# XiYe20/NPVP

Hardware: AMD Instinct MI355X
Metric: predictor train frames/sec (higher is better)
Workload: dtype f32 (two-term fp16 split of amax-scaled operands, 3 MFMAs per product, fp32 accumulate: fp32-grade; small GEMMs: three-term bf16 split)

## Files before the change

include/npvp_hip.h:

```cpp
#ifndef NPVP_HIP_H
#define NPVP_HIP_H
#include <stddef.h>
#ifdef __cplusplus
extern "C" {
#endif

typedef struct ihipStream_t* npvp_stream_t;

int npvp_version(void);
const char* npvp_last_error(void);
long long npvp_launch_count(void);
void* npvp_stream_create_low_priority(int* least, int* greatest);
int npvp_stream_destroy(void* stream);
void* npvp_event_create(void);
int npvp_event_record(void* event, void* stream);
float npvp_event_elapsed_ms(void* event0, void* event1);
int npvp_event_destroy(void* event);

long long npvp_graph_node_counts(void* graph, long long* counts, long long* memset_bytes, int max_memsets);

long long npvp_gemm_workspace_bytes(int M, int N, int K);
int npvp_gemm_kernel_id(int a_kc, int b_kc, int M, int N, int K, int precision, int has_planes);
int npvp_gemm_route(int a_kc, int b_kc, int M, int N, int K, int precision, int has_planes, int plain_epilogue, int* out4);
int npvp_gemm_f32(int a_kc, int b_kc, int M, int N, int K, const float* A, long long lda, const float* B, long long ldb,
// ... 67 lines not shown
int npvp_layernorm_bwd_reduce_job(const void* workspace, float* dw, float* db, long long rows, int C, int accumulate, void* job);
int npvp_frameln_act_bwd_reduce_job(const void* workspace, float* dw, float* db, int frames, int per_frame, int accumulate, void* job);
int npvp_mlpdw_mid_bwd_reduce_job(const void* workspace, float* gw, float* gb, int frames, int Ch, void* job);
int npvp_sum_rows_multi(const void* jobs, int n, npvp_stream_t stream);

int npvp_layernorm_nchw_fwd(const float* x, const float* w, const float* b, float* out_nchw, float* mean, float* rstd, int frames,
                            int P, int C, float eps, int relu, npvp_stream_t stream);

int npvp_frame_stats(const float* x, const float* add, float* mean, float* rstd, int frames, int T, int per_frame,
                     float eps, npvp_stream_t stream);
int npvp_posfuse_fwd(const float* x, const float* add, const float* beta, const float* gamma, float* y, float* mean,
                     float* rstd, int N, int T, int per_frame, float eps, float* y_amax, npvp_stream_t stream);
int npvp_ln_posfuse_fwd(const float* x, const float* lw, const float* lb, float ln_eps, float* y1, float* ln_mean, float* ln_rstd,
                        const float* add, const float* beta, const float* gamma, float* fused, float* pf_mean, float* pf_rstd,
                        int N, int T, int P, int C, float pf_eps, float* y1_amax, float* fused_amax, npvp_stream_t stream);
int npvp_posfuse_bwd_fused(int N, int T, int per_frame);
int npvp_posfuse_bwd(const float* dy, const float* x, const float* add, const float* gamma, const float* mean,
                     const float* rstd, float* du, float* dyxh, float* dbeta, float* dgamma, int N, int T, int per_frame,
                     int accumulate, void* workspace, long long ws_bytes , npvp_stream_t stream);

int npvp_posfuse_instance_fwd(const float* x, const float* add, const float* beta, const float* gamma, float* y, float* mean,
                              float* rstd, int N, int T, int P, int C, float eps, float* y_amax, npvp_stream_t stream);
int npvp_posfuse_instance_bwd(const float* dy, const float* x, const float* add, const float* gamma, const float* mean,
                              const float* rstd, float* du, float* dyxh, int N, int T, int P, int C, npvp_stream_t stream);

int npvp_frameln_act_fwd(const float* h, const float* mean, const float* rstd, const float* w, const float* b,
                         const float* res, float* out, int frames, int per_frame, float drop_p, unsigned int salt,
                         float dp_p, unsigned int dp_salt, int frames_per_sample, const unsigned long long* seed,
                         float* out_amax, npvp_stream_t stream);
long long npvp_frameln_act_bwd_workspace_bytes(int frames, int per_frame);
// ... 56 lines not shown
int npvp_im2col3x3(const float* in, float* out, int frames, int H, int W, int C, int col2im, npvp_stream_t stream);
long long npvp_dwconv3x3_wgrad_workspace_bytes(int frames, int Ch);
int npvp_dwconv3x3_wgrad(const float* a, const float* dout, float* dwt_db, int frames, int H, int W, int Ch,
                         void* workspace, long long ws_bytes, npvp_stream_t stream);

int npvp_attn_fwd(const float* q, long long ld_q, const float* k, long long ld_k, const float* v, long long ld_v, float* o,
                  long long ld_o, int mode, int dim0, int P, int W, int ws, int Tq, int Tk, int heads, int head_dim,
                  int mask_mode, float drop_p, const unsigned long long* seed, unsigned int salt, float* o_amax,
                  npvp_stream_t stream);
int npvp_attn_bwd(const float* q, long long ld_q, const float* k, long long ld_k, const float* v, long long ld_v,
                  const float* go, long long ld_o, float* dq, long long ld_dq, float* dk, long long ld_dk, float* dv,
                  long long ld_dv, int mode, int dim0, int P, int W, int ws, int Tq, int Tk, int heads, int head_dim,
                  int mask_mode, float drop_p, const unsigned long long* seed, unsigned int salt, float* dq_amax,
                  float* dk_amax , float* dv_amax,
                  npvp_stream_t stream);
int npvp_attn_long_fwd(const float* q, long long ld_q, const float* k, long long ld_k, const float* v, long long ld_v, float* o,
                       long long ld_o, int mode, int dim0, int P, int W, int ws, int Tq, int Tk, int heads, int head_dim,
                       int mask_mode, float drop_p, const unsigned long long* seed, unsigned int salt, float* o_amax,
                       npvp_stream_t stream);
long long npvp_attn_long_bwd_workspace_bytes(int mode, int dim0, int P, int W, int ws, int Tq, int Tk, int heads);
int npvp_attn_long_bwd(const float* q, long long ld_q, const float* k, long long ld_k, const float* v, long long ld_v,
                       const float* go, long long ld_o, float* dq, long long ld_dq, float* dk, long long ld_dk, float* dv,
                       long long ld_dv, int mode, int dim0, int P, int W, int ws, int Tq, int Tk, int heads, int head_dim,
                       int mask_mode, float drop_p, const unsigned long long* seed, unsigned int salt, float* dq_amax,
                       float* dk_amax , float* dv_amax, void* workspace, long long ws_bytes,
                       npvp_stream_t stream);

int npvp_reparam_samples(const float* mu, const float* logvar, float* z, float* eps_out, long long numel, int S,
                         long long sample_base, const unsigned long long* seed, unsigned int salt, npvp_stream_t stream);
int npvp_attn_samples_fwd(const float* q, long long ld_q, const float* k, long long ld_k, const float* v, long long ld_v, float* o,
// ... 155 lines not shown
```

npvp_amd/csrc/attn.hip:

```cpp
#include <cstdio>

#include "common.h"

namespace npvp {

constexpr int HD = 64;
constexpr int LDT = 68;

struct AttnParams {
  const float* q; const float* k; const float* v; const float* go;
  float* o;
  float* dq; float* dk; float* dv;
  long long ld_q, ld_k, ld_v, ld_o;
  long long ld_dq, ld_dk, ld_dv;
  int mode, heads, L, S;
  int P, W, ws, nww, nwin;
  int Tq, Tk;
  int mask_mode;
  float scale;
  unsigned int drop_thresh; float drop_inv_keep; unsigned int salt;
  const unsigned long long* seed;
  long long total;
  float* o_amax; float* dq_amax; float* dk_amax; float* dv_amax;
};

struct AttnRows { int mode, a, b, P, W, ws; float inv_ws; };
__device__ __forceinline__ AttnRows attn_rows(const AttnParams& p, unsigned int g) {
  AttnRows r;
  r.mode = p.mode; r.P = p.P; r.W = p.W; r.ws = p.ws; r.b = 0; r.inv_ws = 0.f;
  if (p.mode == 0) {
    const unsigned int f = g / (unsigned int)p.nwin, win = g - f * (unsigned int)p.nwin;
    const unsigned int qh = win / (unsigned int)p.nww, qw = win - qh * (unsigned int)p.nww;
    r.a = (int)(f * (unsigned int)p.P + qh * (unsigned int)(p.ws * p.W) + qw * (unsigned int)p.ws);
    r.inv_ws = 1.f / (float)p.ws;
  } else {
    const unsigned int n = g / (unsigned int)p.P;
    r.a = (int)n; r.b = (int)(g - n * (unsigned int)p.P);
  }
// ... 13 lines not shown
}
__device__ __forceinline__ float attn_keep(const AttnParams& p, unsigned long long seed, unsigned long long wid, int L, int S, int q, int j) {
  return drop_scale(seed, p.salt, (wid * L + q) * S + j, p.drop_thresh, p.drop_inv_keep);
}
struct AttnWave { int head; AttnRows g; int L, S, Tq, Tk; unsigned long long seed; };
__device__ __forceinline__ AttnWave attn_wave(const AttnParams& p, unsigned int wid) {
  AttnWave aw;
  aw.head = (int)(wid % (unsigned int)p.heads);
  aw.g = attn_rows(p, wid / (unsigned int)p.heads);
  aw.L = p.L; aw.S = p.S;
  aw.Tq = p.mode == 1 ? p.Tq : 0; aw.Tk = p.mode == 1 ? p.Tk : 0;
  aw.seed = (p.seed && p.drop_thresh) ? *p.seed : 0ull;
  return aw;
}

typedef float f32x4_t __attribute__((ext_vector_type(4)));
#define NPVP_MFMA16(A, B, C) __builtin_amdgcn_mfma_f32_16x16x4f32((A), (B), (C), 0, 0, 0)

struct AttnTileR { float v[16]; };
struct AttnTileG { float4 v[4]; };

__device__ __forceinline__ void attn_load_r(AttnTileR& t, const float* src, long long ld, const AttnParams& p, const AttnRows& g,
                                            int nrows, int Tn, int head, int n, int c, int blk) {
  const int r = min(16 * blk + n, nrows - 1);
  const float* q = src + attn_row(g, r, Tn) * ld + head * HD + 16 * c;
#pragma unroll
  for (int s4 = 0; s4 < 4; ++s4) {
    const float4 x = ld4(q + 4 * s4);
    t.v[4 * s4 + 0] = x.x; t.v[4 * s4 + 1] = x.y; t.v[4 * s4 + 2] = x.z; t.v[4 * s4 + 3] = x.w;
  }
// ... 18 lines not shown
    }
  }
}
__device__ __forceinline__ float blk_of(const float4& x, int b) { return b == 0 ? x.x : b == 1 ? x.y : b == 2 ? x.z : x.w; }

__device__ __forceinline__ void attn_mm_rows(f32x4_t (&acc)[4], const float (&a)[4], const AttnTileG& gt) {
#pragma unroll
  for (int b = 0; b < 4; ++b) {
#pragma unroll
    for (int i = 0; i < 4; ++i) acc[b] = NPVP_MFMA16(a[i], blk_of(gt.v[i], b), acc[b]);
  }
}
__device__ __forceinline__ void attn_zero(f32x4_t (&acc)[4]) {
#pragma unroll
  for (int b = 0; b < 4; ++b) acc[b] = f32x4_t{0.f, 0.f, 0.f, 0.f};
}
__device__ __forceinline__ f32x4_t attn_mm_d(const AttnTileR& a, const AttnTileR& b) {
  f32x4_t acc = {0.f, 0.f, 0.f, 0.f};
#pragma unroll
  for (int s = 0; s < 16; ++s) acc = NPVP_MFMA16(a.v[s], b.v[s], acc);
  return acc;
}
__device__ __forceinline__ float quad_max(float v) { v = fmaxf(v, __shfl_xor(v, 16, 64)); return fmaxf(v, __shfl_xor(v, 32, 64)); }
__device__ __forceinline__ float quad_sum(float v) { v += __shfl_xor(v, 16, 64); return v + __shfl_xor(v, 32, 64); }

template <int NK, bool MASK, bool BWD, class KT>
__device__ __forceinline__ void attn_row_block(float (&sc)[NK][4], float (*dp)[4], float& mx, float& inv, KT&& ktile, const AttnTileR& qr,
                                               const AttnTileR* vr, const AttnTileR* gr, float scale, int mask_mode, int L, int S, int q, int c) {
  mx = -INFINITY;
#pragma unroll
// ... 73 lines not shown
    for (int i = 0; i < 4; ++i) {
      sc[kb][i] *= inv;
      if constexpr (STAGED) pm[kb][i] = sc[kb][i] * m[kb][i];
      dp[kb][i] = STAGED ? mul_rounded(dp[kb][i], m[kb][i]) : dp[kb][i] * m[kb][i];
      rs += dp[kb][i] * sc[kb][i];
    }
  return quad_sum(rs);
}

template <int NQ, int NK>
__global__ __launch_bounds__(256) void attn_fwd_mfma_kernel(AttnParams p) {
  const int lane = threadIdx.x & 63, n = lane & 15, c = lane >> 4;
  const long long wid = (long long)blockIdx.x * 4 + (threadIdx.x >> 6);
  if (wid >= p.total) return;
  const AttnWave aw = attn_wave(p, (unsigned int)wid);
  AttnTileR kr[NK];
  AttnTileG vg[NK];
  float am_o = 0.f;
  const unsigned int pk_o = amax_peek_wave(p.o_amax);
#pragma unroll
  for (int kb = 0; kb < NK; ++kb) {
    attn_load_r(kr[kb], p.k, p.ld_k, p, aw.g, aw.S, aw.Tk, aw.head, n, c, kb);
    attn_load_g(vg[kb], p.v, p.ld_v, p, aw.g, aw.S, aw.Tk, aw.head, n, c, kb);
  }
#pragma unroll
  for (int qb = 0; qb < NQ; ++qb) attn_fwd_qblock<NK, false>(p, aw, aw.g, wid, kr, vg, qb, n, c, am_o);
  amax_slot_commit(p.o_amax, am_o, pk_o);
}

template <int NQ, int NK>
// ... 18 lines not shown
  for (int s = (int)ck * chunk; s < s_end; ++s) {
    gq.a = s * nclip + aw.g.a;
#pragma unroll
    for (int qb = 0; qb < NQ; ++qb) attn_fwd_qblock<NK, true>(p, aw, gq, 0ull, kr, vg, qb, n, c, am_o);
  }
  amax_slot_commit(p.o_amax, am_o, pk_o);
}

template <int NQ, int NK>
__global__ __launch_bounds__(256) void attn_bwd_mfma_kernel(AttnParams p) {
  const int lane = threadIdx.x & 63, n = lane & 15, c = lane >> 4;
  const long long wid = (long long)blockIdx.x * 4 + (threadIdx.x >> 6);
  if (wid >= p.total) return;
  const AttnWave aw = attn_wave(p, (unsigned int)wid);
  const AttnRows& g = aw.g; const int head = aw.head, L = aw.L, S = aw.S, Tq = aw.Tq, Tk = aw.Tk;
  AttnTileR kr[NK], vr[NK];
#pragma unroll
  for (int kb = 0; kb < NK; ++kb) {
    attn_load_r(kr[kb], p.k, p.ld_k, p, g, S, Tk, head, n, c, kb);
    attn_load_r(vr[kb], p.v, p.ld_v, p, g, S, Tk, head, n, c, kb);
  }
  float mxs[NQ], invs[NQ], rss[NQ], am_q = 0.f, am_k = 0.f, am_v = 0.f;
  const unsigned int pk_q = amax_peek_wave(p.dq_amax), pk_k = amax_peek_wave(p.dk_amax), pk_v = amax_peek_wave(p.dv_amax);
  AttnTileR qr, gr;
#pragma unroll
  for (int qb = 0; qb < NQ; ++qb) {
    attn_load_r(qr, p.q, p.ld_q, p, g, L, Tq, head, n, c, qb);
    attn_load_r(gr, p.go, p.ld_o, p, g, L, Tq, head, n, c, qb);
    AttnTileG kg[NK];
#pragma unroll
// ... 575 lines not shown
                         long long ld_v, float* o, long long ld_o, float* o_amax) {
  if (ld_q % 4 || ld_k % 4 || ld_v % 4 || ld_o % 4) return attn_fail(who, "row strides must be multiples of 4");
  p.q = q; p.k = k; p.v = v; p.o = o; p.ld_q = ld_q; p.ld_k = ld_k; p.ld_v = ld_v; p.ld_o = ld_o; p.o_amax = o_amax;
  return NPVP_OK;
}
static int attn_bind_bwd(AttnParams& p, const char* who, const float* q, long long ld_q, const float* k, long long ld_k, const float* v,
                         long long ld_v, const float* go, long long ld_o, float* dq, long long ld_dq, float* dk, long long ld_dk, float* dv,
                         long long ld_dv, float* dq_amax, float* dk_amax, float* dv_amax) {
  if (ld_q % 4 || ld_k % 4 || ld_v % 4 || ld_o % 4 || ld_dq % 4 || ld_dk % 4 || ld_dv % 4) return attn_fail(who, "row strides must be multiples of 4");
  p.q = q; p.k = k; p.v = v; p.go = go; p.dq = dq; p.dk = dk; p.dv = dv;
  p.ld_q = ld_q; p.ld_k = ld_k; p.ld_v = ld_v; p.ld_o = ld_o; p.ld_dq = ld_dq; p.ld_dk = ld_dk; p.ld_dv = ld_dv;
  p.dq_amax = dq_amax; p.dk_amax = dk_amax; p.dv_amax = dv_amax;
  return NPVP_OK;
}

}

using namespace npvp;

extern "C" int npvp_attn_fwd(const float* q, long long ld_q, const float* k, long long ld_k, const float* v, long long ld_v,
                             float* o, long long ld_o, int mode, int dim0, int P, int W, int ws, int Tq, int Tk, int heads,
                             int head_dim, int mask_mode, float drop_p, const unsigned long long* seed, unsigned int salt,
                             float* o_amax, hipStream_t stream) {
  AttnParams p = {};
  if (const int rc = attn_setup(p, "attn", mode, heads, head_dim, dim0, P, W, ws, Tq, Tk, mask_mode, drop_p, seed, salt)) return rc;
  NPVP_CHECK_ARG(dim0 > 0, "attn: empty batch");
  if (const int rc = attn_bind_fwd(p, "attn", q, ld_q, k, ld_k, v, ld_v, o, ld_o, o_amax)) return rc;
  const dim3 mg((unsigned)((p.total + 3) / 4)), mb(256);
  const int nq = (p.L + 15) / 16, nk = (p.S + 15) / 16;
  if (nq > 2 || nk > 2) {
    const size_t lds = (size_t)2 * p.S * HD * sizeof(float);
    if (lds > 64 * 1024 && hipFuncSetAttribute((const void*)attn_fwd_generic_kernel, hipFuncAttributeMaxDynamicSharedMemorySize, (int)lds) != hipSuccess)
      return attn_fail("attn", "could not reserve LDS for the generic kernel", NPVP_ERR_LAUNCH);
    NPVP_LAUNCH(attn_fwd_generic_kernel, dim3((unsigned)p.total), dim3(GEN_THREADS), lds, stream, p);
    NPVP_CHECK_LAUNCH();
    return NPVP_OK;
  }
  if (nq == 1 && nk == 1) NPVP_LAUNCH((attn_fwd_mfma_kernel<1, 1>), mg, mb, 0, stream, p);
  else if (nq == 1) NPVP_LAUNCH((attn_fwd_mfma_kernel<1, 2>), mg, mb, 0, stream, p);
  else if (nk == 1) NPVP_LAUNCH((attn_fwd_mfma_kernel<2, 1>), mg, mb, 0, stream, p);
  else NPVP_LAUNCH((attn_fwd_mfma_kernel<2, 2>), mg, mb, 0, stream, p);
// ... 27 lines not shown
  const dim3 mg((unsigned)((p.total + 3) / 4)), mb(256);
  const int nq = (Tq + 15) / 16, nk = (Tk + 15) / 16, ck = (int)chunk;
  if (nq == 1 && nk == 1) NPVP_LAUNCH((attn_samples_fwd_mfma_kernel<1, 1>), mg, mb, 0, stream, p, S, N, ck);
  else if (nq == 1) NPVP_LAUNCH((attn_samples_fwd_mfma_kernel<1, 2>), mg, mb, 0, stream, p, S, N, ck);
  else if (nk == 1) NPVP_LAUNCH((attn_samples_fwd_mfma_kernel<2, 1>), mg, mb, 0, stream, p, S, N, ck);
  else NPVP_LAUNCH((attn_samples_fwd_mfma_kernel<2, 2>), mg, mb, 0, stream, p, S, N, ck);
  NPVP_CHECK_LAUNCH();
  return NPVP_OK;
}

extern "C" int npvp_attn_bwd(const float* q, long long ld_q, const float* k, long long ld_k, const float* v, long long ld_v,
                             const float* go, long long ld_o, float* dq, long long ld_dq, float* dk, long long ld_dk,
                             float* dv, long long ld_dv, int mode, int dim0, int P, int W, int ws, int Tq, int Tk,
                             int heads, int head_dim, int mask_mode, float drop_p, const unsigned long long* seed,
                             unsigned int salt, float* dq_amax, float* dk_amax, float* dv_amax, hipStream_t stream) {
  AttnParams p = {};
  if (const int rc = attn_setup(p, "attn", mode, heads, head_dim, dim0, P, W, ws, Tq, Tk, mask_mode, drop_p, seed, salt)) return rc;
  NPVP_CHECK_ARG(dim0 > 0, "attn_bwd: empty batch");
  if (const int rc = attn_bind_bwd(p, "attn_bwd", q, ld_q, k, ld_k, v, ld_v, go, ld_o, dq, ld_dq, dk, ld_dk, dv, ld_dv, dq_amax, dk_amax, dv_amax))
    return rc;
  const size_t staged1_lds = (size_t)(2 * p.L + p.S) * LDT * sizeof(float) + 2 * 16 * LDX * sizeof(float);
  const dim3 mg((unsigned)((p.total + 3) / 4)), mb(256);
  const int nq = (p.L + 15) / 16, nk = (p.S + 15) / 16;
  if (nq > 2 || nk > 2) {
    const size_t lds = ((size_t)2 * (p.L + p.S) * HD + 3 * (size_t)p.L) * sizeof(float);
    if (lds > 64 * 1024 && hipFuncSetAttribute((const void*)attn_bwd_generic_kernel, hipFuncAttributeMaxDynamicSharedMemorySize, (int)lds) != hipSuccess)
      return attn_fail("attn_bwd", "could not reserve LDS for the generic kernel", NPVP_ERR_LAUNCH);
    NPVP_LAUNCH(attn_bwd_generic_kernel, dim3((unsigned)p.total), dim3(GEN_THREADS), lds, stream, p);
    NPVP_CHECK_LAUNCH();
    return NPVP_OK;
  }
  if (nq == 1 && nk == 1) NPVP_LAUNCH((attn_bwd_mfma_kernel<1, 1>), mg, mb, 0, stream, p);
  else if (nq == 1) NPVP_LAUNCH((attn_bwd_mfma_kernel<1, 2>), mg, mb, 0, stream, p);
// ... 61 lines not shown
```

npvp_amd/csrc/norm.hip:

```cpp
#include "partials.h"
#include <cstring>
#include <cstdlib>

namespace npvp {

template <int NV>
__global__ __launch_bounds__(256) void ln_fwd_kernel(const float* __restrict__ x, const float* __restrict__ w,
                                                     const float* __restrict__ b, float* __restrict__ y,
                                                     float* __restrict__ mean, float* __restrict__ rstd, long long rows,
                                                     float eps, int relu, float* __restrict__ amax) {
  constexpr int C = NV * 256;
  __shared__ float ared[4];
  const unsigned int peek = amax_peek_block(amax);
  const int lane = threadIdx.x & 63;
  float4 ww[NV], bb[NV];
#pragma unroll
  for (int i = 0; i < NV; ++i) { ww[i] = ld4(w + (i * 64 + lane) * 4); bb[i] = ld4(b + (i * 64 + lane) * 4); }
  float am = 0.f;
  for (long long row = (long long)blockIdx.x * 4 + (threadIdx.x >> 6); row < rows; row += (long long)gridDim.x * 4) {
    float4 v[NV];
    float s = 0.f;
#pragma unroll
    for (int i = 0; i < NV; ++i) {
      v[i] = ld4(x + row * C + (i * 64 + lane) * 4);
// ... 279 lines not shown
    if (gt) { const float4 g = ld4(gt + e); o.x *= 1.f + g.x; o.y *= 1.f + g.y; o.z *= 1.f + g.z; o.w *= 1.f + g.w; }
    const float4 b = ld4(bt + e);
    o.x += b.x; o.y += b.y; o.z += b.z; o.w += b.w;
    st4(yf + e, o);
    am = amax4(am, o);
  }
  amax_slot_commit_block(amax, am, ared, peek);
}

__global__ __launch_bounds__(1024) void ln_posfuse_fwd_frame_kernel(const float* __restrict__ x, const float* __restrict__ lw,
                                                                    const float* __restrict__ lb, float ln_eps, float* __restrict__ y1,
                                                                    float* __restrict__ ln_mean, float* __restrict__ ln_rstd,
                                                                    const float* __restrict__ add, const float* __restrict__ beta,
                                                                    const float* __restrict__ gamma, float* __restrict__ fused,
                                                                    float* __restrict__ pf_mean, float* __restrict__ pf_rstd, int T,
                                                                    float pf_eps, float* __restrict__ amax1, float* __restrict__ amax2) {
  constexpr int C = 512, P = 64, PF = P * C;
  __shared__ float red[16];
  __shared__ float ared1[16];
  __shared__ float ared2[16];
  const unsigned int peek1 = amax_peek_block(amax1), peek2 = amax_peek_block(amax2);
  const int f = blockIdx.x, n = f / T, t = f - n * T;
  const int lane = threadIdx.x & 63, wave = threadIdx.x >> 6;
  float4 ww[2], bb[2];
#pragma unroll
  for (int i = 0; i < 2; ++i) { ww[i] = ld4(lw + (i * 64 + lane) * 4); bb[i] = ld4(lb + (i * 64 + lane) * 4); }
  float4 v[4][2];
  float am1 = 0.f, su = 0.f;
#pragma unroll
  for (int r = 0; r < 4; ++r) {
    const int row = wave * 4 + r;
    const long long base = (long long)f * PF + (long long)row * C;
    float s = 0.f;
#pragma unroll
    for (int i = 0; i < 2; ++i) { v[r][i] = ld4(x + base + (i * 64 + lane) * 4); s += (v[r][i].x + v[r][i].y) + (v[r][i].z + v[r][i].w); }
    const float mu = wave_sum(s) * (1.f / C);
    float q = 0.f;
#pragma unroll
// ... 573 lines not shown
    return NPVP_OK;
  }
  NPVP_LAUNCH(frame_stats_kernel, dim3(frames), dim3(512), 0, stream, x, add, mean, rstd, T, per_frame, eps);
  NPVP_CHECK_LAUNCH();
  const long long total4 = (long long)frames * per_frame / 4;
  NPVP_LAUNCH(posfuse_apply_kernel, dim3(ew_blocks(total4, 256)), dim3(256), 0, stream, x, add, beta, gamma,
                     (const float*)mean, (const float*)rstd, y, T, per_frame, total4, amax);
  NPVP_CHECK_LAUNCH();
  return NPVP_OK;
}

extern "C" int npvp_ln_posfuse_fwd(const float* x, const float* lw, const float* lb, float ln_eps, float* y1, float* ln_mean,
                                   float* ln_rstd, const float* add, const float* beta, const float* gamma, float* fused,
                                   float* pf_mean, float* pf_rstd, int N, int T, int P, int C, float pf_eps, float* y1_amax,
                                   float* fused_amax, hipStream_t stream) {
  NPVP_CHECK_ARG(N > 0 && T > 0 && P == 64 && C == 512, "ln_posfuse_fwd: frames of 64 token rows x 512 channels only");
  NPVP_CHECK_ARG(x && lw && lb && y1 && ln_mean && ln_rstd && beta && fused && pf_mean && pf_rstd, "ln_posfuse_fwd: null argument");
  NPVP_LAUNCH(ln_posfuse_fwd_frame_kernel, dim3(N * T), dim3(1024), 0, stream, x, lw, lb, ln_eps, y1, ln_mean, ln_rstd, add,
                     beta, gamma, fused, pf_mean, pf_rstd, T, pf_eps, y1_amax, fused_amax);
  NPVP_CHECK_LAUNCH();
  return NPVP_OK;
}

extern "C" int npvp_posfuse_bwd_fused(int N, int T, int per_frame) {
  if (per_frame % 1024 != 0) return 0;
  const long long blocks = (long long)T * (per_frame / 1024);
  return (blocks >= 128 || N <= 16) ? 1 : 0;
}

extern "C" int npvp_posfuse_bwd(const float* dy, const float* x, const float* add, const float* gamma, const float* mean,
                                const float* rstd, float* du, float* dyxh, float* dbeta, float* dgamma, int N, int T,
                                int per_frame, int accumulate, void* workspace, long long ws_bytes, hipStream_t stream) {
  const int frames = N * T;
  NPVP_CHECK_ARG(N > 0 && T > 0 && per_frame % 4 == 0, "posfuse_bwd: bad shape");
// ... 170 lines not shown
```

npvp_amd/ops.py:

```python
import contextlib
import functools
import os
from collections import namedtuple

import torch

from ._lib import lib, check
from . import sched as _S
from .sched import (_p, _ptr, _stream, _ws, AmaxSlot, GemmProbe, HbmProbe, ProbeEvent, AuxStream, StepContext, current, use, scoped,
                    remember, rng, GradSink, WgradStream, WgradChain, ReduceQueue, RangeGuard)


def amax_of(t, slot=None):
    if slot is not None:
        return slot
    for cand in (t, t._base):
        tag = getattr(cand, "_npvp_amax", None) if cand is not None else None
        if tag is not None and tag[1] == cand._version:
            return tag[0]
    s = AmaxSlot.new(t.device)
    t2 = t if t.dim() == 2 else t.reshape(-1, t.shape[-1])
    if t2.stride(1) != 1:
        t2 = t2.contiguous()
    check(lib().npvp_amax(_ptr(t2), t2.shape[0], t2.shape[1], t2.stride(0), _ptr(s), _stream()), "npvp_amax")
# ... 1067 lines not shown
    return (cfg.ws * cfg.ws, cfg.ws * cfg.ws) if cfg.mode == 0 else (cfg.Tq, cfg.Tk)


def _attn_groups(cfg):
    return cfg.dim0 * (cfg.P // (cfg.ws * cfg.ws)) if cfg.mode == 0 else cfg.dim0 * cfg.P


def _attn_long(cfg):
    return max(_attn_len(cfg)) >= ATTN_LONG_MIN


def _attn_fwd_entry(cfg):
    return (lib().npvp_attn_long_fwd, "npvp_attn_long_fwd") if _attn_long(cfg) else (lib().npvp_attn_fwd, "npvp_attn_fwd")


def _attn_fwd(q, k, v, o, cfg):
    hd = o.shape[1] // cfg.heads
    seed = _S._cur.rng.seed_for(q.device, cfg.drop)
    if DropRecorder.sites is not None and cfg.drop.on:
        L_, S_ = _attn_len(cfg)
        DropRecorder.note(cfg.drop, "elem", _attn_groups(cfg) * cfg.heads * L_ * S_)
    slot = _new_slot(q.device)
    fn, what = _attn_fwd_entry(cfg)
    check(fn(_ptr(q), q.stride(0), _ptr(k), k.stride(0), _ptr(v), v.stride(0), _ptr(o), o.stride(0),
             cfg.mode, cfg.dim0, cfg.P, cfg.W, cfg.ws, cfg.Tq, cfg.Tk, cfg.heads, hd, cfg.mask_mode,
             cfg.drop.p, _ptr(seed), cfg.drop.salt, _ptr(slot), _stream()), what)
    tag_amax(o, slot)


ATTN_SAMPLES_MAX = 32


def _attn_samples_fwd(q, k, v, o, cfg, S, sample_chunk=0):
    if cfg.mode != 1 or cfg.mask_mode != 0 or cfg.drop.on:
        raise ValueError("_attn_samples_fwd: temporal geometry without mask and dropout only")
    hd = o.shape[1] // cfg.heads
    slot = _new_slot(q.device)
    if max(cfg.Tq, cfg.Tk) <= ATTN_SAMPLES_MAX:
        check(lib().npvp_attn_samples_fwd(_ptr(q), q.stride(0), _ptr(k), k.stride(0), _ptr(v), v.stride(0), _ptr(o), o.stride(0),
                                          S, cfg.dim0, cfg.P, cfg.Tq, cfg.Tk, cfg.heads, hd, sample_chunk, _ptr(slot), _stream()),
              "npvp_attn_samples_fwd")
    else:
        fn, what = _attn_fwd_entry(cfg)
        rows = cfg.dim0 * cfg.Tq * cfg.P
        for s in range(S):
            check(fn(q.data_ptr() + 4 * s * rows * q.stride(0), q.stride(0), _ptr(k), k.stride(0), _ptr(v), v.stride(0),
                     o.data_ptr() + 4 * s * rows * o.stride(0), o.stride(0), 1, cfg.dim0, cfg.P, cfg.W, 0, cfg.Tq, cfg.Tk, cfg.heads,
                     hd, 0, 0.0, None, 0, _ptr(slot), _stream()), what)
    tag_amax(o, slot)


def _attn_bwd(q, k, v, go, dq, dk, dv, cfg, packed=None):
    hd = go.shape[1] // cfg.heads
    seed = _S._cur.rng.seed_for(q.device, cfg.drop)
    sq = _new_slot(q.device)
    sk = sq if packed is not None else _new_slot(q.device)
    sv = _new_slot(q.device)
    args = (_ptr(q), q.stride(0), _ptr(k), k.stride(0), _ptr(v), v.stride(0), _ptr(go), go.stride(0),
            _ptr(dq), dq.stride(0), _ptr(dk), dk.stride(0), _ptr(dv), dv.stride(0), cfg.mode, cfg.dim0,
            cfg.P, cfg.W, cfg.ws, cfg.Tq, cfg.Tk, cfg.heads, hd, cfg.mask_mode, cfg.drop.p, _ptr(seed),
            cfg.drop.salt, _ptr(sq), _ptr(sk), _ptr(sv))
    if _attn_long(cfg):
        ws, wsn = _ws(lib().npvp_attn_long_bwd_workspace_bytes(cfg.mode, cfg.dim0, cfg.P, cfg.W, cfg.ws, cfg.Tq, cfg.Tk, cfg.heads),
                      q.device)
        check(lib().npvp_attn_long_bwd(*args, _ptr(ws), wsn, _stream()), "npvp_attn_long_bwd")
    else:
        check(lib().npvp_attn_bwd(*args, _stream()), "npvp_attn_bwd")
    if packed is not None:
        tag_amax(packed, sq)
    else:
        tag_amax(dq, sq); tag_amax(dk, sk)
    tag_amax(dv, sv)


class _AttnPacked(_Function):

    @staticmethod
    def forward(ctx, qk, v, cfg):
        remember(ctx)
        _chk(qk, v)
        C = v.shape[1]
        o = torch.empty_like(v)
# ... 275 lines not shown
        else:
            gdww = torch.empty(hid, 1, 3, 3, dtype=torch.float32, device=dev)
            check(L.npvp_transpose(_ptr(dwtb), _ptr(gdww), 1, 9, hid, _stream()), "npvp_transpose")
            gdwb = dwtb[9]
        dh1, gn1w, gn1b = _fln_bwd(da1, h1, stats[0], stats[1], n1w, n1b, frames, 64 * hid, NO_DROP, NO_DROP, 1, s_n1,
                                      psum=psum, nparts=nparts, skip=ctx.skip)
        del da1
        dx, gw1, gb1 = linear_bwd(dh1, x, w1, True if has_b1 else None, s_fc1, skip=ctx.skip)
        return (dx, dout if has_res else None, gw1, gb1, gn1w, gn1b, gdww, gdwb, gn2w, gn2b, gw2, gb2, gn3w, gn3b,
                None, None, None, None)


MID_BWD_N2 = True
DROP_PATH_SKIP = True
WGRAD_ROW_SKIP = True


def mlpdwbn_fused_supported(R, C, hid, Co, H, W):
    return (GEMM_PRECISION in (4, 6) and H == 8 and W == 8 and R % 64 == 0 and hid % 512 == 0 and Co % 128 == 0 and hid % 128 == 0
            and C % 32 == 0)


def mlpdwbn(x, res, w1, b1, n1w, n1b, dww, dwb, n2w, n2b, w2, b2, n3w, n3b, frames, T, p_drop, p_dp):
    return _MlpDwbn.apply(x, res, w1, b1, n1w, n1b, dww, dwb, n2w, n2b, w2, b2, n3w, n3b, frames, T, p_drop, p_dp)


def _raw_ln_fwd(x2, w, b, eps, relu=0):
    rows, C = x2.shape
    y = torch.empty_like(x2)
    st = torch.empty(2, rows, dtype=torch.float32, device=x2.device)
# ... 23 lines not shown


def _raw_posfuse_fwd(x, add, beta, gamma, N, T):
    PF = x.numel() // (N * T)
    y = torch.empty_like(x)
    st = torch.empty(2, N * T, dtype=torch.float32, device=x.device)
    slot = _new_slot(x.device)
    check(lib().npvp_posfuse_fwd(_ptr(x), _ptr(add), _ptr(beta), _ptr(gamma), _ptr(y), _row(st, 0), _row(st, 1), N, T, PF, 1e-5,
                                 _ptr(slot), _stream()), "npvp_posfuse_fwd")
    return tag_amax(y, slot), st


LN_POSFUSE_ONE_KERNEL = True


def _raw_ln_posfuse_fwd(x2, lw, lb, eps, add, beta, gamma, N, T):
    rows, C = x2.shape
    if not (LN_POSFUSE_ONE_KERNEL and C == 512 and rows == N * T * 64):
        x1, lst = _raw_ln_fwd(x2, lw, lb, eps)
        fused, pst = _raw_posfuse_fwd(x1, add, beta, gamma, N, T)
        return x1, lst, fused, pst
    x1, fused = torch.empty_like(x2), torch.empty_like(x2)
    lst = torch.empty(2, rows, dtype=torch.float32, device=x2.device)
    pst = torch.empty(2, N * T, dtype=torch.float32, device=x2.device)
    s1, s2 = _new_slot(x2.device), _new_slot(x2.device)
    check(lib().npvp_ln_posfuse_fwd(_ptr(x2), _ptr(lw), _ptr(lb), eps, _ptr(x1), _row(lst, 0), _row(lst, 1), _ptr(add), _ptr(beta),
                                    _ptr(gamma), _ptr(fused), _row(pst, 0), _row(pst, 1), N, T, 64, C, 1e-5, _ptr(s1), _ptr(s2),
                                    _stream()), "npvp_ln_posfuse_fwd")
    return tag_amax(x1, s1), lst, tag_amax(fused, s2), pst


def _raw_posfuse_bwd(dy, x, add, beta_shape, gamma, st, N, T, want_add, sinks=(None, None, None)):
    PF = x.numel() // (N * T)
    du, dbeta, dgamma = _posfuse_bwd_call(dy, x, add, gamma, st, N, T, PF, beta_shape, True, gamma is not None,
                                          sinks[0], sinks[1])
    dadd = None
    if add is not None and want_add:
        if sinks[2] is not None:
            buf, acc = sinks[2].target(add.shape, x.device)
            reduce_mid(du.view(N, T, PF), out=buf.view(N, PF), accumulate=acc)
        else:
            dadd = reduce_mid(du.view(N, T, PF)).view(add.shape)
    return du, dadd, dbeta, dgamma
# ... 188 lines not shown
    tail = _RowTail(x.shape[0])
    return grid_cut(linear(grid_pad(x, tail), w, b), tail)


class _SelfAttnSublayer(_Function):

    @staticmethod
    def forward(ctx, x, lw, lb, eps, beta, gamma, add, wqk, bqk, wv, bv, wo, bo, cfg, drop, N, T):
        remember(ctx)
        _chk(x, lw, lb, beta, gamma, add, wqk, bqk, wv, bv, wo, bo)
        C = x.shape[-1]
        x2 = _c(x).reshape(-1, C)
        beta_c = _c(beta)
        gamma_c = None if gamma is None else _c(gamma)
        add_c = None if add is None else _c(add)
        x1, lst, fused, pst = _raw_ln_posfuse_fwd(x2, lw, lb, eps, add_c, beta_c, gamma_c, N, T)
        if cfg.tiles:
            qk = linear_fwd(fused, wqk, bqk)
            v = linear_fwd(x1, wv, bv)
            o = torch.empty_like(v)
            _attn_fwd(qk[:, :C], qk[:, C:], v, o, cfg)
        else:
            fused = _raw_grid_pad(fused, cfg)
            qk = linear_fwd(fused, wqk, bqk)
            v = linear_fwd(_raw_grid_pad(x1, cfg), wv, bv)
            o_p = torch.empty_like(v)
            _attn_fwd(qk[:, :C], qk[:, C:], v, o_p, cfg)
            o = _raw_grid_cut(o_p, cfg, want_amax=True)
        y = linear_fwd(o, wo, bo, residual=x2, drop=drop)
        ctx.save_for_backward(x2, x1, lst, fused, pst, qk, v, o, lw, lb, gamma_c, add_c, wqk, bqk, wv, bv, wo, bo)
        ctx.act_sinks = (ActSink.of(beta), ActSink.of(gamma), ActSink.of(add))
        ctx.cfg = (cfg, drop, N, T, x.shape, beta.shape)
        ctx.sinks = (_ln_sink(lw, lb), _wb_sink(wqk, bqk), _wb_sink(wv, bv), _wb_sink(wo, bo))
        return y.view(x.shape)

    @scoped
    def backward(ctx, dy):
        x2, x1, lst, fused, pst, qk, v, o, lw, lb, gamma, add, wqk, bqk, wv, bv, wo, bo = ctx.saved_tensors
        cfg, drop, N, T, xshape, beta_shape = ctx.cfg
        s_ln, s_qk, s_v, s_o = ctx.sinks
        C = x2.shape[1]
        dy2 = _c(dy).reshape(-1, C)
        dz, ad = masked_grad(dy2, drop, wo)
        skip = SampleSkip.of(skip_roles("self_attn", DROP_PATH_SKIP, WGRAD_ROW_SKIP), drop, drop.g1, drop.g2, dy2.shape[0]) if cfg.tiles else NO_SKIP
        do, gwo, gbo = linear_bwd(dz, o, wo, bo, s_o, a_drop=ad, skip=skip)
        if not cfg.tiles:
            do = _raw_grid_pad(do, cfg, want_amax=False)
        dqk, dv = torch.empty_like(qk), torch.empty_like(v)
        _attn_bwd(qk[:, :C], qk[:, C:], v, do, dqk[:, :C], dqk[:, C:], dv, cfg, packed=dqk)
        if not cfg.tiles:
            _zero_tail(cfg, dqk, dv)
        dfused, gwqk, gbqk = linear_bwd(dqk, fused, wqk, bqk, s_qk, skip=skip)
        if not cfg.tiles:
            dfused = _raw_grid_cut(dfused, cfg)
        du, dadd, dbeta, dgamma = _raw_posfuse_bwd(dfused, x1, add, beta_shape, gamma, pst, N, T, ctx.needs_input_grad[6], ctx.act_sinks)
        if cfg.tiles:
            dx1, gwv, gbv = linear_bwd(dv, x1, wv, bv, s_v, residual=du, skip=skip)
        else:
            dx1, gwv, gbv = linear_bwd(dv, _raw_grid_pad(x1, cfg), wv, bv, s_v)
            dx1 = _raw_grid_cut(dx1, cfg, addend=du)
        dx, glw, glb = _raw_ln_bwd(dx1, x2, lw, lb, lst, dy2, s_ln, probe=True)
        return (dx.view(xshape), glw, glb, None, dbeta, dgamma, dadd, gwqk, gbqk, gwv, gbv, gwo, gbo, None, None, None, None)


# ... 829 lines not shown
```

Baseline: 8573.

## Skip LN-posfuse and attention work for drop-path-dropped samples in self-attention

Threads a per-sample frame-skip mask (derived from the drop-path RNG) into the fused LN+posfuse forward kernel and the small-window attention forward and backward kernels. Frames belonging to samples whose residual branch is dropped write zeros instead of computing normalisation, attention, and attention gradients. This removes compute whose output is multiplied by zero by drop-path anyway. It adds RNG-seed plumbing and a per-wave branch, and relies on the skip mask matching the drop-path mask exactly. Zeroed LN stats could also affect the saved tensors used in backward.

```diff
diff --git a/include/npvp_hip.h b/include/npvp_hip.h
--- a/include/npvp_hip.h
+++ b/include/npvp_hip.h
@@ -105,6 +105,10 @@
 int npvp_ln_posfuse_fwd(const float* x, const float* lw, const float* lb, float ln_eps, float* y1, float* ln_mean, float* ln_rstd,
                         const float* add, const float* beta, const float* gamma, float* fused, float* pf_mean, float* pf_rstd,
                         int N, int T, int P, int C, float pf_eps, float* y1_amax, float* fused_amax, npvp_stream_t stream);
+int npvp_ln_posfuse_fwd_skip(const float* x, const float* lw, const float* lb, float ln_eps, float* y1, float* ln_mean, float* ln_rstd,
+                             const float* add, const float* beta, const float* gamma, float* fused, float* pf_mean, float* pf_rstd,
+                             int N, int T, int P, int C, float pf_eps, float* y1_amax, float* fused_amax, float skip_p,
+                             unsigned int skip_salt, int skip_fps, const unsigned long long* seed, npvp_stream_t stream);
 int npvp_posfuse_bwd_fused(int N, int T, int per_frame);
 int npvp_posfuse_bwd(const float* dy, const float* x, const float* add, const float* gamma, const float* mean,
                      const float* rstd, float* du, float* dyxh, float* dbeta, float* dgamma, int N, int T, int per_frame,
@@ -191,6 +195,16 @@
                   int mask_mode, float drop_p, const unsigned long long* seed, unsigned int salt, float* dq_amax,
                   float* dk_amax , float* dv_amax,
                   npvp_stream_t stream);
+int npvp_attn_fwd_skip(const float* q, long long ld_q, const float* k, long long ld_k, const float* v, long long ld_v, float* o,
+                       long long ld_o, int mode, int dim0, int P, int W, int ws, int Tq, int Tk, int heads, int head_dim,
+                       int mask_mode, float drop_p, const unsigned long long* seed, unsigned int salt, float* o_amax,
+                       float skip_p, unsigned int skip_salt, int skip_fps, npvp_stream_t stream);
+int npvp_attn_bwd_skip(const float* q, long long ld_q, const float* k, long long ld_k, const float* v, long long ld_v,
+                       const float* go, long long ld_o, float* dq, long long ld_dq, float* dk, long long ld_dk, float* dv,
+                       long long ld_dv, int mode, int dim0, int P, int W, int ws, int Tq, int Tk, int heads, int head_dim,
+                       int mask_mode, float drop_p, const unsigned long long* seed, unsigned int salt, float* dq_amax,
+                       float* dk_amax, float* dv_amax, float skip_p, unsigned int skip_salt, int skip_fps,
+                       npvp_stream_t stream);
 int npvp_attn_long_fwd(const float* q, long long ld_q, const float* k, long long ld_k, const float* v, long long ld_v, float* o,
                        long long ld_o, int mode, int dim0, int P, int W, int ws, int Tq, int Tk, int heads, int head_dim,
                        int mask_mode, float drop_p, const unsigned long long* seed, unsigned int salt, float* o_amax,
diff --git a/npvp_amd/csrc/attn.hip b/npvp_amd/csrc/attn.hip
--- a/npvp_amd/csrc/attn.hip
+++ b/npvp_amd/csrc/attn.hip
@@ -22,6 +22,7 @@
   const unsigned long long* seed;
   long long total;
   float* o_amax; float* dq_amax; float* dk_amax; float* dv_amax;
+  FrameSkip skip;
 };
 
 struct AttnRows { int mode, a, b, P, W, ws; float inv_ws; };
@@ -65,6 +66,12 @@
   return aw;
 }
 
+__device__ __forceinline__ bool attn_wave_dropped(const AttnParams& p, long long wid) {
+  if (!p.skip.thresh) return false;
+  const unsigned int w = (unsigned int)__builtin_amdgcn_readfirstlane((int)wid);
+  return frame_skipped(p.skip, frame_skip_seed(p.skip), (long long)(w / (unsigned int)(p.heads * p.nwin)));
+}
+
 typedef float f32x4_t __attribute__((ext_vector_type(4)));
 #define NPVP_MFMA16(A, B, C) __builtin_amdgcn_mfma_f32_16x16x4f32((A), (B), (C), 0, 0, 0)
 
@@ -113,6 +120,12 @@
 __device__ __forceinline__ void attn_zero(f32x4_t (&acc)[4]) {
 #pragma unroll
   for (int b = 0; b < 4; ++b) acc[b] = f32x4_t{0.f, 0.f, 0.f, 0.f};
+}
+__device__ __forceinline__ void attn_store_zero(float* dst, long long ld, const AttnParams& p, const AttnRows& g, int nrows, int head, int n, int c) {
+  f32x4_t z[4];
+  attn_zero(z);
+  float am = 0.f;
+  attn_store_d(z, dst, ld, p, g, nrows, 0, head, n, c, 0, am);
 }
 __device__ __forceinline__ f32x4_t attn_mm_d(const AttnTileR& a, const AttnTileR& b) {
   f32x4_t acc = {0.f, 0.f, 0.f, 0.f};
@@ -216,6 +229,9 @@
   const long long wid = (long long)blockIdx.x * 4 + (threadIdx.x >> 6);
   if (wid >= p.total) return;
   const AttnWave aw = attn_wave(p, (unsigned int)wid);
+  if constexpr (NQ == 1 && NK == 1) {
+    if (attn_wave_dropped(p, wid)) { attn_store_zero(p.o, p.ld_o, p, aw.g, aw.L, aw.head, n, c); return; }
+  }
   AttnTileR kr[NK];
   AttnTileG vg[NK];
   float am_o = 0.f;
@@ -264,6 +280,14 @@
   if (wid >= p.total) return;
   const AttnWave aw = attn_wave(p, (unsigned int)wid);
   const AttnRows& g = aw.g; const int head = aw.head, L = aw.L, S = aw.S, Tq = aw.Tq, Tk = aw.Tk;
+  if constexpr (NQ == 1 && NK == 1) {
+    if (attn_wave_dropped(p, wid)) {
+      attn_store_zero(p.dq, p.ld_dq, p, g, L, head, n, c);
+      attn_store_zero(p.dk, p.ld_dk, p, g, S, head, n, c);
+      attn_store_zero(p.dv, p.ld_dv, p, g, S, head, n, c);
+      return;
+    }
+  }
   AttnTileR kr[NK], vr[NK];
 #pragma unroll
   for (int kb = 0; kb < NK; ++kb) {
@@ -869,6 +893,15 @@
   return NPVP_OK;
 }
 
+static int attn_bind_skip(AttnParams& p, const char* who, int mode, int dim0, float skip_p, unsigned int skip_salt, int skip_fps,
+                          const unsigned long long* seed) {
+  if (skip_p == 0.f) return NPVP_OK;
+  if (skip_p < 0.f || skip_p >= 1.f || !seed) return attn_fail(who, "bad skip arguments (skip_p in [0, 1), a device seed)");
+  if (mode != 0 || skip_fps <= 0 || dim0 % skip_fps != 0) return attn_fail(who, "a sample skip needs spatial mode and whole samples of skip_fps frames");
+  if (p.L <= 16 && p.S <= 16) p.skip = make_frame_skip(skip_p, skip_salt, skip_fps, seed);
+  return NPVP_OK;
+}
+
 }
 
 using namespace npvp;
@@ -877,9 +910,18 @@
                              float* o, long long ld_o, int mode, int dim0, int P, int W, int ws, int Tq, int Tk, int heads,
                              int head_dim, int mask_mode, float drop_p, const unsigned long long* seed, unsigned int salt,
                              float* o_amax, hipStream_t stream) {
+  return npvp_attn_fwd_skip(q, ld_q, k, ld_k, v, ld_v, o, ld_o, mode, dim0, P, W, ws, Tq, Tk, heads, head_dim, mask_mode, drop_p, seed, salt,
+                            o_amax, 0.f, 0u, 1, stream);
+}
+
+extern "C" int npvp_attn_fwd_skip(const float* q, long long ld_q, const float* k, long long ld_k, const float* v, long long ld_v,
+                                  float* o, long long ld_o, int mode, int dim0, int P, int W, int ws, int Tq, int Tk, int heads,
+                                  int head_dim, int mask_mode, float drop_p, const unsigned long long* seed, unsigned int salt,
+                                  float* o_amax, float skip_p, unsigned int skip_salt, int skip_fps, hipStream_t stream) {
   AttnParams p = {};
   if (const int rc = attn_setup(p, "attn", mode, heads, head_dim, dim0, P, W, ws, Tq, Tk, mask_mode, drop_p, seed, salt)) return rc;
   NPVP_CHECK_ARG(dim0 > 0, "attn: empty batch");
+  if (const int rc = attn_bind_skip(p, "attn", mode, dim0, skip_p, skip_salt, skip_fps, seed)) return rc;
   if (const int rc = attn_bind_fwd(p, "attn", q, ld_q, k, ld_k, v, ld_v, o, ld_o, o_amax)) return rc;
   const dim3 mg((unsigned)((p.total + 3) / 4)), mb(256);
   const int nq = (p.L + 15) / 16, nk = (p.S + 15) / 16;
@@ -937,9 +979,20 @@
                              float* dv, long long ld_dv, int mode, int dim0, int P, int W, int ws, int Tq, int Tk,
                              int heads, int head_dim, int mask_mode, float drop_p, const unsigned long long* seed,
                              unsigned int salt, float* dq_amax, float* dk_amax, float* dv_amax, hipStream_t stream) {
+  return npvp_attn_bwd_skip(q, ld_q, k, ld_k, v, ld_v, go, ld_o, dq, ld_dq, dk, ld_dk, dv, ld_dv, mode, dim0, P, W, ws, Tq, Tk, heads, head_dim,
+                            mask_mode, drop_p, seed, salt, dq_amax, dk_amax, dv_amax, 0.f, 0u, 1, stream);
+}
+
+extern "C" int npvp_attn_bwd_skip(const float* q, long long ld_q, const float* k, long long ld_k, const float* v, long long ld_v,
+                                  const float* go, long long ld_o, float* dq, long long ld_dq, float* dk, long long ld_dk,
+                                  float* dv, long long ld_dv, int mode, int dim0, int P, int W, int ws, int Tq, int Tk,
+                                  int heads, int head_dim, int mask_mode, float drop_p, const unsigned long long* seed,
+                                  unsigned int salt, float* dq_amax, float* dk_amax, float* dv_amax, float skip_p,
+                                  unsigned int skip_salt, int skip_fps, hipStream_t stream) {
   AttnParams p = {};
   if (const int rc = attn_setup(p, "attn", mode, heads, head_dim, dim0, P, W, ws, Tq, Tk, mask_mode, drop_p, seed, salt)) return rc;
   NPVP_CHECK_ARG(dim0 > 0, "attn_bwd: empty batch");
+  if (const int rc = attn_bind_skip(p, "attn_bwd", mode, dim0, skip_p, skip_salt, skip_fps, seed)) return rc;
   if (const int rc = attn_bind_bwd(p, "attn_bwd", q, ld_q, k, ld_k, v, ld_v, go, ld_o, dq, ld_dq, dk, ld_dk, dv, ld_dv, dq_amax, dk_amax, dv_amax))
     return rc;
   const size_t staged1_lds = (size_t)(2 * p.L + p.S) * LDT * sizeof(float) + 2 * 16 * LDX * sizeof(float);
diff --git a/npvp_amd/csrc/norm.hip b/npvp_amd/csrc/norm.hip
--- a/npvp_amd/csrc/norm.hip
+++ b/npvp_amd/csrc/norm.hip
@@ -317,14 +317,28 @@
                                                                     const float* __restrict__ add, const float* __restrict__ beta,
                                                                     const float* __restrict__ gamma, float* __restrict__ fused,
                                                                     float* __restrict__ pf_mean, float* __restrict__ pf_rstd, int T,
-                                                                    float pf_eps, float* __restrict__ amax1, float* __restrict__ amax2) {
+                                                                    float pf_eps, float* __restrict__ amax1, float* __restrict__ amax2,
+                                                                    FrameSkip skip) {
   constexpr int C = 512, P = 64, PF = P * C;
   __shared__ float red[16];
   __shared__ float ared1[16];
   __shared__ float ared2[16];
-  const unsigned int peek1 = amax_peek_block(amax1), peek2 = amax_peek_block(amax2);
   const int f = blockIdx.x, n = f / T, t = f - n * T;
   const int lane = threadIdx.x & 63, wave = threadIdx.x >> 6;
+  if (frame_skipped(skip, frame_skip_seed(skip), f)) {
+    const float4 z = make_float4(0.f, 0.f, 0.f, 0.f);
+#pragma unroll
+    for (int r = 0; r < 4; ++r) {
+      const int row = wave * 4 + r;
+      const long long base = (long long)f * PF + (long long)row * C;
+#pragma unroll
+      for (int i = 0; i < 2; ++i) { st4(y1 + base + (i * 64 + lane) * 4, z); st4(fused + base + (i * 64 + lane) * 4, z); }
+      if (lane == 0) { ln_mean[(long long)f * P + row] = 0.f; ln_rstd[(long long)f * P + row] = 0.f; }
+    }
+    if (threadIdx.x == 0) { pf_mean[f] = 0.f; pf_rstd[f] = 0.f; }
+    return;
+  }
+  const unsigned int peek1 = amax_peek_block(amax1), peek2 = amax_peek_block(amax2);
   float4 ww[2], bb[2];
 #pragma unroll
   for (int i = 0; i < 2; ++i) { ww[i] = ld4(lw + (i * 64 + lane) * 4); bb[i] = ld4(lb + (i * 64 + lane) * 4); }
@@ -928,10 +942,21 @@
                                    float* ln_rstd, const float* add, const float* beta, const float* gamma, float* fused,
                                    float* pf_mean, float* pf_rstd, int N, int T, int P, int C, float pf_eps, float* y1_amax,
                                    float* fused_amax, hipStream_t stream) {
+  return npvp_ln_posfuse_fwd_skip(x, lw, lb, ln_eps, y1, ln_mean, ln_rstd, add, beta, gamma, fused, pf_mean, pf_rstd, N, T, P, C, pf_eps,
+                                  y1_amax, fused_amax, 0.f, 0u, 1, nullptr, stream);
+}
+
+extern "C" int npvp_ln_posfuse_fwd_skip(const float* x, const float* lw, const float* lb, float ln_eps, float* y1, float* ln_mean,
+                                        float* ln_rstd, const float* add, const float* beta, const float* gamma, float* fused,
+                                        float* pf_mean, float* pf_rstd, int N, int T, int P, int C, float pf_eps, float* y1_amax,
+                                        float* fused_amax, float skip_p, unsigned int skip_salt, int skip_fps,
+                                        const unsigned long long* seed, hipStream_t stream) {
   NPVP_CHECK_ARG(N > 0 && T > 0 && P == 64 && C == 512, "ln_posfuse_fwd: frames of 64 token rows x 512 channels only");
   NPVP_CHECK_ARG(x && lw && lb && y1 && ln_mean && ln_rstd && beta && fused && pf_mean && pf_rstd, "ln_posfuse_fwd: null argument");
+  NPVP_CHECK_ARG(skip_p == 0.f || (skip_p > 0.f && skip_p < 1.f && seed && skip_fps > 0), "ln_posfuse_fwd: bad skip arguments");
   NPVP_LAUNCH(ln_posfuse_fwd_frame_kernel, dim3(N * T), dim3(1024), 0, stream, x, lw, lb, ln_eps, y1, ln_mean, ln_rstd, add,
-                     beta, gamma, fused, pf_mean, pf_rstd, T, pf_eps, y1_amax, fused_amax);
+                     beta, gamma, fused, pf_mean, pf_rstd, T, pf_eps, y1_amax, fused_amax,
+                     make_frame_skip(skip_p, skip_salt, skip_fps, seed));
   NPVP_CHECK_LAUNCH();
   return NPVP_OK;
 }
diff --git a/npvp_amd/ops.py b/npvp_amd/ops.py
--- a/npvp_amd/ops.py
+++ b/npvp_amd/ops.py
@@ -1105,17 +1105,20 @@
     return (lib().npvp_attn_long_fwd, "npvp_attn_long_fwd") if _attn_long(cfg) else (lib().npvp_attn_fwd, "npvp_attn_fwd")
 
 
-def _attn_fwd(q, k, v, o, cfg):
+def _attn_fwd(q, k, v, o, cfg, skip=NO_SKIP.frame):
     hd = o.shape[1] // cfg.heads
-    seed = _S._cur.rng.seed_for(q.device, cfg.drop)
+    seed = _S._cur.rng.seed_for(q.device, cfg.drop, skip)
     if DropRecorder.sites is not None and cfg.drop.on:
         L_, S_ = _attn_len(cfg)
         DropRecorder.note(cfg.drop, "elem", _attn_groups(cfg) * cfg.heads * L_ * S_)
     slot = _new_slot(q.device)
-    fn, what = _attn_fwd_entry(cfg)
-    check(fn(_ptr(q), q.stride(0), _ptr(k), k.stride(0), _ptr(v), v.stride(0), _ptr(o), o.stride(0),
-             cfg.mode, cfg.dim0, cfg.P, cfg.W, cfg.ws, cfg.Tq, cfg.Tk, cfg.heads, hd, cfg.mask_mode,
-             cfg.drop.p, _ptr(seed), cfg.drop.salt, _ptr(slot), _stream()), what)
+    args = (_ptr(q), q.stride(0), _ptr(k), k.stride(0), _ptr(v), v.stride(0), _ptr(o), o.stride(0),
+            cfg.mode, cfg.dim0, cfg.P, cfg.W, cfg.ws, cfg.Tq, cfg.Tk, cfg.heads, hd, cfg.mask_mode,
+            cfg.drop.p, _ptr(seed), cfg.drop.salt, _ptr(slot))
+    if _attn_long(cfg):
+        check(lib().npvp_attn_long_fwd(*args, _stream()), "npvp_attn_long_fwd")
+    else:
+        check(lib().npvp_attn_fwd_skip(*args, skip.p, skip.salt, skip.fps, _stream()), "npvp_attn_fwd_skip")
     tag_amax(o, slot)
 
 
@@ -1141,9 +1144,9 @@
     tag_amax(o, slot)
 
 
-def _attn_bwd(q, k, v, go, dq, dk, dv, cfg, packed=None):
+def _attn_bwd(q, k, v, go, dq, dk, dv, cfg, packed=None, skip=NO_SKIP.frame):
     hd = go.shape[1] // cfg.heads
-    seed = _S._cur.rng.seed_for(q.device, cfg.drop)
+    seed = _S._cur.rng.seed_for(q.device, cfg.drop, skip)
     sq = _new_slot(q.device)
     sk = sq if packed is not None else _new_slot(q.device)
     sv = _new_slot(q.device)
@@ -1156,7 +1159,7 @@
                       q.device)
         check(lib().npvp_attn_long_bwd(*args, _ptr(ws), wsn, _stream()), "npvp_attn_long_bwd")
     else:
-        check(lib().npvp_attn_bwd(*args, _stream()), "npvp_attn_bwd")
+        check(lib().npvp_attn_bwd_skip(*args, skip.p, skip.salt, skip.fps, _stream()), "npvp_attn_bwd_skip")
     if packed is not None:
         tag_amax(packed, sq)
     else:
@@ -1462,6 +1465,14 @@
 MID_BWD_N2 = True
 DROP_PATH_SKIP = True
 WGRAD_ROW_SKIP = True
+ATTN_DROP_PATH_SKIP = True
+
+
+def attn_skip(on, cfg, drop, rows, precision=6, strict=False):
+    if not (on and cfg.mode == 0 and cfg.tiles and drop.on and drop.mode == 1 and drop.g1 * drop.g2 == rows and drop.g1 % cfg.P == 0
+            and precision == 6 and not strict):
+        return NO_SKIP.frame
+    return FrameSkip(drop.p, drop.salt, drop.g1 // cfg.P)
 
 
 def mlpdwbn_fused_supported(R, C, hid, Co, H, W):
@@ -1515,7 +1526,7 @@
 LN_POSFUSE_ONE_KERNEL = True
 
 
-def _raw_ln_posfuse_fwd(x2, lw, lb, eps, add, beta, gamma, N, T):
+def _raw_ln_posfuse_fwd(x2, lw, lb, eps, add, beta, gamma, N, T, skip=NO_SKIP.frame):
     rows, C = x2.shape
     if not (LN_POSFUSE_ONE_KERNEL and C == 512 and rows == N * T * 64):
         x1, lst = _raw_ln_fwd(x2, lw, lb, eps)
@@ -1525,9 +1536,10 @@
     lst = torch.empty(2, rows, dtype=torch.float32, device=x2.device)
     pst = torch.empty(2, N * T, dtype=torch.float32, device=x2.device)
     s1, s2 = _new_slot(x2.device), _new_slot(x2.device)
-    check(lib().npvp_ln_posfuse_fwd(_ptr(x2), _ptr(lw), _ptr(lb), eps, _ptr(x1), _row(lst, 0), _row(lst, 1), _ptr(add), _ptr(beta),
-                                    _ptr(gamma), _ptr(fused), _row(pst, 0), _row(pst, 1), N, T, 64, C, 1e-5, _ptr(s1), _ptr(s2),
-                                    _stream()), "npvp_ln_posfuse_fwd")
+    check(lib().npvp_ln_posfuse_fwd_skip(_ptr(x2), _ptr(lw), _ptr(lb), eps, _ptr(x1), _row(lst, 0), _row(lst, 1), _ptr(add), _ptr(beta),
+                                         _ptr(gamma), _ptr(fused), _row(pst, 0), _row(pst, 1), N, T, 64, C, 1e-5, _ptr(s1), _ptr(s2),
+                                         skip.p, skip.salt, skip.fps, _ptr(_S._cur.rng.seed_for(x2.device, skip)), _stream()),
+          "npvp_ln_posfuse_fwd_skip")
     return tag_amax(x1, s1), lst, tag_amax(fused, s2), pst
 
 
@@ -1746,12 +1758,13 @@
         beta_c = _c(beta)
         gamma_c = None if gamma is None else _c(gamma)
         add_c = None if add is None else _c(add)
-        x1, lst, fused, pst = _raw_ln_posfuse_fwd(x2, lw, lb, eps, add_c, beta_c, gamma_c, N, T)
+        ctx.askip = askip = attn_skip(ATTN_DROP_PATH_SKIP, cfg, drop, x2.shape[0], GEMM_PRECISION, _S._cur.range_guard.strict)
+        x1, lst, fused, pst = _raw_ln_posfuse_fwd(x2, lw, lb, eps, add_c, beta_c, gamma_c, N, T, skip=askip)
         if cfg.tiles:
             qk = linear_fwd(fused, wqk, bqk)
             v = linear_fwd(x1, wv, bv)
             o = torch.empty_like(v)
-            _attn_fwd(qk[:, :C], qk[:, C:], v, o, cfg)
+            _attn_fwd(qk[:, :C], qk[:, C:], v, o, cfg, skip=askip)
         else:
             fused = _raw_grid_pad(fused, cfg)
             qk = linear_fwd(fused, wqk, bqk)
@@ -1779,7 +1792,7 @@
         if not cfg.tiles:
             do = _raw_grid_pad(do, cfg, want_amax=False)
         dqk, dv = torch.empty_like(qk), torch.empty_like(v)
-        _attn_bwd(qk[:, :C], qk[:, C:], v, do, dqk[:, :C], dqk[:, C:], dv, cfg, packed=dqk)
+        _attn_bwd(qk[:, :C], qk[:, C:], v, do, dqk[:, :C], dqk[:, C:], dv, cfg, packed=dqk, skip=ctx.askip)
         if not cfg.tiles:
             _zero_tail(cfg, dqk, dv)
         dfused, gwqk, gbqk = linear_bwd(dqk, fused, wqk, bqk, s_qk, skip=skip)
```

New measurement: 8572. About the same (-0.0%).
